# QuantEcon/dynamic_factor_models

Measured on NVIDIA H100. Metric: EM iters/sec (N=200,r=8,T=500), higher is better.
Workload: dtype f64

## Files before the change

dynamic_factor_models_b200/csrc/dfm_api.cu:

```cuda
#include "../../include/dfm_b200.h"
#include "dfm_common.cuh"
#include "dfm_kernels_np.cuh"
#include "dfm_kernels_em.cuh"
#include "dfm_kernels_emb.cuh"
#include "dfm_kernels_ss.cuh"
#include "dfm_kernels_fused.cuh"
#include "dfm_kernels_fused2.cuh"
#include "dfm_kernels_als_masked.cuh"
#include "dfm_kernels_rep.cuh"
#include "dfm_kernels_inst.cuh"
#include <algorithm>
#include <new>
#include <thread>
#include <type_traits>
#include <vector>
#ifndef DFM_EMU
#include <dlfcn.h>
#else
#include <map>
#include <mutex>
#endif

#ifdef DFM_EMU
typedef int cudaError_t;
// ... 24 lines not shown
static inline cudaError_t cudaFree(void* p) { free(p); return 0; }
static inline cudaError_t cudaMemcpyAsync(void* d, const void* s, size_t n, cudaMemcpyKind, cudaStream_t) { memcpy(d, s, n); return 0; }
static inline cudaError_t cudaMemsetAsync(void* d, int v, size_t n, cudaStream_t) { memset(d, v, n); return 0; }
static inline cudaError_t cudaMemcpy2DAsync(void* d, size_t dp, const void* s, size_t sp, size_t w, size_t rows, cudaMemcpyKind, cudaStream_t) {
  for (size_t j = 0; j < rows; ++j) memcpy((char*)d + j * dp, (const char*)s + j * sp, w);
  return 0;
}
static inline cudaError_t cudaStreamCreate(cudaStream_t* s) { *s = nullptr; return 0; }
static inline cudaError_t cudaStreamDestroy(cudaStream_t) { return 0; }
static inline cudaError_t cudaStreamSynchronize(cudaStream_t) { return 0; }
static inline cudaError_t cudaSetDevice(int) { return 0; }
static inline cudaError_t cudaGetDeviceCount(int* n) { *n = 1; return 0; }
static inline cudaError_t cudaGetLastError() { cudaError_t e = g_emu_last_err; g_emu_last_err = cudaSuccess; return e; }
static inline const char* cudaGetErrorString(cudaError_t e) {
  return e == cudaErrorInvalidConfiguration ? "emu: launch past a device limit (grid, block or shared memory)"
       : e == cudaErrorInvalidValue ? "emu: shared-memory attribute past the device limit" : "emu";
}
#define DFM_SET_SMEM(kern, bytes) emu_set_smem((const void*)(kern), (size_t)(bytes))
#else
#define DFM_SET_SMEM(kern, bytes) cudaFuncSetAttribute(kern, cudaFuncAttributeMaxDynamicSharedMemorySize, (int)(bytes))
#endif

using namespace dfm;

struct ProfRec { const char* name; 
#ifndef DFM_EMU
  cudaEvent_t e0, e1;
#endif
};

struct dfm_handle {
  int device;
  int nsm;
  cudaStream_t stream;
  cudaStream_t copy_stream;
  cudaStream_t d2h_stream;
  int* done_host; int* done_dev; size_t done_cap;
  int* pinned_one;
  bool own_stream;
  char* ws;
  size_t ws_bytes;
  long long launches;
  int profile;
  std::vector<ProfRec>* prof;
  char err[256];
};

namespace {

const size_t kMaxSmem = 220 * 1024;
const int kMaxReadyChunks = 4096;
const int kMaxGridBatch = 65535;

struct Arena {
  char* base; size_t off;
  explicit Arena(char* b) : base(b), off(0) {}
  template <typename Tp> Tp* get(size_t n) {
    size_t bytes = (n * sizeof(Tp) + 255) & ~(size_t)255;
    Tp* p = base ? reinterpret_cast<Tp*>(base + off) : nullptr;
    off += bytes;
    return p;
  }
};

int fail(dfm_handle* h, int code, const char* msg) {
  if (h) { snprintf(h->err, sizeof(h->err), "%s", msg); }
// ... 92 lines not shown
  cuuint64_t strides[1] = {(cuuint64_t)T * 8};
  cuuint32_t box[2] = {F2_TS, 8 * F2_SBS}, es[2] = {1, 1};
  CUresult rc = fn(out, CU_TENSOR_MAP_DATA_TYPE_FLOAT64, 2, (void*)X, dims, strides, box, es, CU_TENSOR_MAP_INTERLEAVE_NONE,
                   CU_TENSOR_MAP_SWIZZLE_NONE, CU_TENSOR_MAP_L2_PROMOTION_L2_256B, CU_TENSOR_MAP_FLOAT_OOB_FILL_NONE);
  if (rc != CUDA_SUCCESS) { snprintf(h->err, sizeof(h->err), "cuTensorMapEncodeTiled failed (%d)", (int)rc); return DFM_ERR_CUDA; }
  return DFM_OK;
#endif
}

template <int Lo, int Hi, typename F>
static auto dispatch(int v, F&& f) {
  if constexpr (Lo == Hi) return f(std::integral_constant<int, Lo>{});
  else {
    if (v == Lo) return f(std::integral_constant<int, Lo>{});
    return dispatch<Lo + 1, Hi>(v, f);
  }
}

template <typename K>
static int resident_grid(const dfm_handle* h, K kern, int threads, size_t smem, int B) {
#ifdef DFM_EMU
  (void)threads;
  DFM_SET_SMEM(kern, smem);
  return std::min(B, h->nsm * 8);
#else
  DFM_SET_SMEM(kern, smem);
  int occ = 1;
  cudaOccupancyMaxActiveBlocksPerMultiprocessor(&occ, kern, threads, smem);
  if (occ < 1) occ = 1;
  return std::min(B, h->nsm * occ);
#endif
}

static int launch_em_fused(dfm_handle* h, const FusedArgs& fa, int r, bool use2) {
  return dispatch<1, 8>(r, [&](auto R) -> int {
    constexpr int RT = decltype(R)::value;
    if (use2) {
      const size_t smem = fused2_smem_doubles<RT>(fa.T, fa.N) * 8;
      const int grid = resident_grid(h, k_em_fused2<RT>, 256, smem, fa.B);
      CUtensorMap tm; int rc = make_panel_tmap(h, fa.X, fa.T, (long long)fa.B * fa.N, &tm); if (rc) return rc;
      L(k_em_fused2<RT>, grid, 1, 256, smem, fa, tm);
    } else {
      const size_t smem = fused_smem_doubles<RT>(fa.T, fa.N) * 8;
      const int grid = resident_grid(h, k_em_fused<RT>, 128, smem, fa.B);
      L(k_em_fused<RT>, grid, 1, 128, smem, fa);
    }
    return DFM_OK;
  });
}

struct EmbPlan {
  bool on; int ncb, ntE, nsE, nper, ntM, tsM, tper;
  double *Bpart, *qpart, *Spart, *sxxpart, *Cpart; int* counters;
  size_t smE, smM;
};
static EmbPlan emb_plan(int T, int N, int r, int batch, int nsm) {
  EmbPlan e{};
  e.on = r <= 32;
  if (!e.on) return e;
  e.ncb = (r + 7) / 8;
  const int target = 2 * nsm;
  e.ntE = (T + EMB_TILE - 1) / EMB_TILE;
  int want = (target + e.ntE * batch - 1) / (e.ntE * batch);
  int ns = std::max((N + EMB_MAXSPLIT - 1) / EMB_MAXSPLIT, std::min(want, (N + 31) / 32));
  e.nper = (((N + ns - 1) / ns) + 3) & ~3;
  e.nsE = (N + e.nper - 1) / e.nper;
  e.ntM = (N + EMB_TILE - 1) / EMB_TILE;
  want = (target + e.ntM * batch - 1) / (e.ntM * batch);
  int ts = std::max(1, std::min(want, (T + 31) / 32));
  e.tper = (((T + ts - 1) / ts) + 3) & ~3;
  e.tsM = (T + e.tper - 1) / e.tper;
  if ((long long)e.nsE * batch > 65535 || (long long)e.tsM * batch > 65535) { e.on = false; return e; }
// ... 118 lines not shown
  int n_missing = batch;
  if (emb.on) {
    L(k_em_count_missing, 1, 1, 128, 48 * 8, d.st, batch, d.active);
    CK(cudaMemcpyAsync(&n_missing, d.active, sizeof(int), cudaMemcpyDeviceToHost, h->stream));
    CK(cudaStreamSynchronize(h->stream));
    CK(cudaMemsetAsync(emb.counters, 0, sizeof(int) * (size_t)batch * (emb.ntE + emb.ntM), h->stream));
  }
  const bool any_missing = n_missing > 0, any_bal = emb.on ? (n_missing < batch) : true;
  const int emb_on = emb.on ? 1 : 0;
  int h_active = batch;
  for (int it = 0; it < mi && h_active > 0; ++it) {
    if (any_missing) L(k_em_contract, nblkC, batch, ntC, ((size_t)(np + r) * ntC + 8) * 8, x, d.L, g.W, d.R, g.logR, g.C, T, N, r, g.Bt, g.qt, g.slr, g.nt, g.Ct, d.st);
    if (any_bal) {
      if (!emb.on) L(k_em_contract_bal, (T + 31) / 32, batch, 256, 8 * 32 * 3 * 8, x, g.W, d.R, g.logR, T, N, r, g.Bt, g.qt, g.slr, g.nt, d.st);
      else emb_launch_E(h, emb, x, g.W, d.R, g.logR, T, N, r, batch, g.Bt, g.qt, g.slr, g.nt, d.st);
    }
    launch_filter_smooth(h, ncl, g, batch, T, r, p, d.A, d.Q, d.P0, d.Fs, d.PsF, d.ll, d.st, mi, o->tol, want_psf);
    if (any_missing || !emb.on) L(k_em_mstep_series, N, batch, 64, (size_t)(2 * np + r + 8) * 8, x, d.Fs, d.PsF, g.Sff, T, N, r, d.L, d.R, d.st, emb_on);
    if (any_bal && emb.on) {
      emb_launch_M(h, emb, x, d.Fs, g.Sff, T, N, r, batch, d.L, d.R, g.W, g.logR, d.st);
      L(k_emb_close, batch, 1, 256, 0, N, r, p, emb.ntM, emb.Cpart, g.C, d.A, g.An, d.Q, g.Qn, d.st, mi, 1);
    }
    if (any_missing || !emb.on) L(k_em_prep, batch, 1, 128, 0, d.L, d.R, N, r, p, g.W, g.logR, g.C, d.A, g.An, d.Q, g.Qn, d.st, mi, 1, emb_on);
    if (o->tol > 0 && ((it & 3) == 3)) {
      L(k_em_count_active, 1, 1, 128, 48 * 8, d.st, batch, d.active);
      CK(cudaMemcpyAsync(&h_active, d.active, sizeof(int), cudaMemcpyDeviceToHost, h->stream));
      CK(cudaStreamSynchronize(h->stream));
    }
  }
  L(k_em_collect, batch, 1, 1, 0, d.st, d.it, d.stat);
  return DFM_OK;
}

static int launch_als_fused2(dfm_handle* h, const AlsFusedArgs& fa, int r) {
  return dispatch<1, 8>(r, [&](auto R) -> int {
    constexpr int RT = decltype(R)::value;
    const size_t smem = als_fused2_smem_doubles<RT>(fa.T, fa.N) * 8;
    const int grid = resident_grid(h, k_als_fused2<RT>, 256, smem, fa.B);
    CUtensorMap tm; int rc = make_panel_tmap(h, fa.Xs, fa.T, (long long)fa.B * fa.N, &tm); if (rc) return rc;
    L(k_als_fused2<RT>, grid, 1, 256, smem, fa, tm);
    return DFM_OK;
  });
}
static void launch_als_masked(dfm_handle* h, const AlsMaskedArgs& fa, int r) {
  dispatch<1, 8>(r, [&](auto R) {
    constexpr int RT = decltype(R)::value;
    const size_t smem = als_masked_smem_doubles<RT>(fa.T, fa.N) * 8;
    const int grid = resident_grid(h, k_als_masked<RT>, 256, smem, fa.B);
    L(k_als_masked<RT>, grid, 1, 256, smem, fa);
  });
}
static bool als_masked_shape_ok(int T, int N, int r) {
  if (r < 1 || r > 8) return false;
  return ((size_t)r * (T | 1) + (size_t)r * (N | 1) + 5 * (size_t)r * r + 48) * 8 <= 100 * 1024;
}
static bool als_fused2_shape_ok(int T, int N, int r) {
  if (r < 1 || r > 8 || T < 4 || (T & 1)) return false;
  return ((size_t)FZ * pad4mod16(T) + (size_t)r * pad4mod16(N) + (size_t)N + 4 * (size_t)r * r + 2 * r + 48 +
          2 * F2_NCW * 72 + (size_t)F2_S * F2_STG + 32) * 8 <= 113 * 1024;
}

static bool fused2_shape_ok(int T, int N, int r, int p) {
  if (p != 1 || r < 1 || r > 8 || T < 4 || (T & 1)) return false;
  size_t need = ((size_t)FZ * pad4mod16(T) + (size_t)r * pad4mod16(N) + 3 * (size_t)N + 30 * (size_t)r * r + 2 * (size_t)r +
                 std::max((size_t)97 * r + (size_t)r * r, (size_t)2 * F2_NCW * 72) + (size_t)F2_S * F2_STG + 106) * 8;
  return need <= 113 * 1024;
}

static bool fused_shape_ok(int T, int N, int r, int p) {
  if (p != 1 || r < 1 || r > 8 || T < 3) return false;
  return ((size_t)FZ * pad4mod16(T) + (size_t)r * pad4mod16(N) + 3 * (size_t)N + 31 * (size_t)r * r + 66 * (size_t)r + 128) * 8 <= kMaxSmem;
// ... 128 lines not shown
    case DFM_ERR_CUDA: return "CUDA error / no device";
    case DFM_ERR_UNSUPPORTED: return "unsupported problem size";
    case DFM_ERR_NCCL: return "NCCL error";
  }
  return "unknown";
}

static void handle_teardown(dfm_handle* h) {
  if (!h) return;
  if (h->stream) cudaStreamSynchronize(h->stream);
  if (h->ws) cudaFree(h->ws);
  if (h->own_stream && h->stream) cudaStreamDestroy(h->stream);
#ifndef DFM_EMU
  if (h->copy_stream) { cudaStreamSynchronize(h->copy_stream); cudaStreamDestroy(h->copy_stream); }
  if (h->pinned_one) cudaFreeHost(h->pinned_one);
  if (h->d2h_stream) { cudaStreamSynchronize(h->d2h_stream); cudaStreamDestroy(h->d2h_stream); }
  if (h->done_host) cudaFreeHost(h->done_host);
  if (h->prof) for (auto& r : *h->prof) { cudaEventDestroy(r.e0); cudaEventDestroy(r.e1); }
#endif
  delete h->prof;
  delete h;
}

int dfm_create_on_stream(int device, void* cuda_stream, dfm_handle** out) {
  if (!out) return DFM_ERR_ARG;
  *out = nullptr;
  int ndev = 0;
  if (cudaGetDeviceCount(&ndev) != cudaSuccess || ndev <= 0 || device < 0 || device >= ndev) return DFM_ERR_CUDA;
  if (cudaSetDevice(device) != cudaSuccess) return DFM_ERR_CUDA;
  dfm_handle* h = new (std::nothrow) dfm_handle();
  if (!h) return DFM_ERR_CUDA;
  h->device = device; h->ws = nullptr; h->ws_bytes = 0; h->launches = 0; h->err[0] = 0;
  h->nsm = 132;
  h->profile = 0; h->prof = new std::vector<ProfRec>();
  h->stream = nullptr; h->own_stream = false;
  h->copy_stream = nullptr; h->pinned_one = nullptr; h->d2h_stream = nullptr; h->done_host = nullptr; h->done_dev = nullptr; h->done_cap = 0;
#ifndef DFM_EMU
  if (cudaDeviceGetAttribute(&h->nsm, cudaDevAttrMultiProcessorCount, device) != cudaSuccess || h->nsm <= 0) { handle_teardown(h); return DFM_ERR_CUDA; }
  if (cudaStreamCreateWithFlags(&h->copy_stream, cudaStreamNonBlocking) != cudaSuccess) { h->copy_stream = nullptr; handle_teardown(h); return DFM_ERR_CUDA; }
  if (cudaStreamCreateWithFlags(&h->d2h_stream, cudaStreamNonBlocking) != cudaSuccess) { h->d2h_stream = nullptr; handle_teardown(h); return DFM_ERR_CUDA; }
  if (cudaHostAlloc((void**)&h->pinned_one, sizeof(int), cudaHostAllocDefault) != cudaSuccess) { h->pinned_one = nullptr; handle_teardown(h); return DFM_ERR_CUDA; }
  *h->pinned_one = 1;
#endif
  if (cuda_stream) { h->stream = (cudaStream_t)cuda_stream; h->own_stream = false; }
  else { if (cudaStreamCreate(&h->stream) != cudaSuccess) { h->stream = nullptr; handle_teardown(h); return DFM_ERR_CUDA; } h->own_stream = true; }
  DFM_SET_SMEM(k_em_filter_smooth, kMaxSmem); DFM_SET_SMEM(k_als_factor, kMaxSmem); DFM_SET_SMEM(k_em_contract, kMaxSmem);
  DFM_SET_SMEM(k_lyapunov, kMaxSmem); DFM_SET_SMEM(k_var, kMaxSmem); DFM_SET_SMEM(k_pca_finish, kMaxSmem);
  DFM_SET_SMEM(k_jacobi, kMaxSmem); DFM_SET_SMEM(k_subspace_eig, kMaxSmem); DFM_SET_SMEM(k_loading, kMaxSmem); DFM_SET_SMEM(k_als_lambda, kMaxSmem);
  if (cudaGetLastError() != cudaSuccess) { handle_teardown(h); return DFM_ERR_CUDA; }
  *out = h;
  return DFM_OK;
}
int dfm_create(int device, dfm_handle** out) { return dfm_create_on_stream(device, nullptr, out); }

int dfm_destroy(dfm_handle* h) {
  if (!h) return DFM_ERR_ARG;
  cudaSetDevice(h->device);
  handle_teardown(h);
  return DFM_OK;
}
int dfm_sync(dfm_handle* h) { if (!h) return DFM_ERR_ARG; CK(cudaStreamSynchronize(h->stream)); return DFM_OK; }
long long dfm_launch_count(const dfm_handle* h) { return h ? h->launches : -1; }
const char* dfm_last_error(const dfm_handle* h) { return h ? h->err : "null handle"; }

int dfm_profile_enable(dfm_handle* h, int on) {
  if (!h) return DFM_ERR_ARG;
  h->profile = on ? 1 : 0;
  return DFM_OK;
}
int dfm_profile_query(dfm_handle* h, const char* name, double* ms, long long* count) {
  if (!h || !ms || !count) return DFM_ERR_ARG;
// ... 753 lines not shown
```

dynamic_factor_models_b200/csrc/dfm_kernels_fused.cuh:

```cuda
#pragma once
#include "dfm_common.cuh"

namespace dfm {

#define FZ 8
#define ZI(t_, i_) ((i_) * Tp + (t_))
#define LI(n_, c_) ((c_) * Np + (n_))
__host__ __device__ inline int pad4mod16(int x) { return x + ((4 - x % 16) + 16) % 16; }

struct FusedArgs {
  const double* X;
  double* Lam;
  double* R;
  double* A;
  double* Q;
  const double* P0;
  double* Fs;
  double* PsF;
  double* loglik;
  int* iters; int* status;
  double* scratch;
  int B, T, N, max_iter;
  double tol;
  const int* ready; int ready_chunk;
  int* done;
  double* P0out;
  int p0_steps;
};
#define FUSED_SCR(R_) (5 * (R_) * (R_) + 1)

__device__ __forceinline__ double w_max(double v) {
#ifndef DFM_EMU
  for (int o = 16; o > 0; o >>= 1) v = fmax(v, __shfl_xor_sync(0xffffffffu, v, o));
#endif
  return v;
}

#ifdef DFM_EMU
#define DFM_HELPER inline
#else
#define DFM_HELPER __device__ __noinline__
#endif
template <int R>
DFM_HELPER void w_gemm(double* C, const double* A, bool ta, const double* B, bool tb) {
#ifndef DFM_EMU
  if (R == 8) {
    const int lane = threadIdx.x & 31, lr = lane >> 2, lc = lane & 3;
    double d0 = 0.0, d1 = 0.0;
#pragma unroll
    for (int kc = 0; kc < 2; ++kc) {
      const int kk = 4 * kc + lc;
      const double av = ta ? A[kk * 8 + lr] : A[lr * 8 + kk];
      const double bv = tb ? B[lr * 8 + kk] : B[kk * 8 + lr];
      asm volatile("mma.sync.aligned.m8n8k4.row.col.f64.f64.f64.f64 {%0,%1}, {%2}, {%3}, {%0,%1};\n"
                   : "+d"(d0), "+d"(d1) : "d"(av), "d"(bv));
    }
    C[lr * 8 + 2 * lc] = d0; C[lr * 8 + 2 * lc + 1] = d1;
    __syncwarp();
    return;
  }
// ... 659 lines not shown
```

dynamic_factor_models_b200/csrc/dfm_kernels_fused2.cuh:

```cuda
#pragma once
#include <algorithm>
#include "dfm_kernels_fused.cuh"
#ifdef DFM_EMU
struct CUtensorMap { char opaque[128]; };
#define DFM_GRID_CONSTANT
#else
#include <cuda.h>
#define DFM_GRID_CONSTANT __grid_constant__
#endif

namespace dfm {

#ifndef F2_SBS
#define F2_SBS 1
#endif
#ifndef F2_S
#define F2_S (4 / F2_SBS)
#endif
#define F2_STG (F2_SBS * 8 * F2_TS)
#ifndef F2_TC
#define F2_TC 132
#endif
#define F2_TS F2_TC
#define F2_NCW 6
#define F2_GPARTS_S 4
#define F2_GPARTS ((R == 8) ? (F2_NCW + 1) : F2_GPARTS_S)
#define F2_NRB (((F2_TC + 7) / 8 + F2_NCW - 1) / F2_NCW)
#define F2_NKC (((F2_TC + 3) / 4 + F2_NCW - 1) / F2_NCW)
static_assert(F2_TC % 16 == 4 || F2_TC % 16 == 12, "ring pitch must be 4 or 12 mod 16");
static_assert(F2_TC <= 256 && (F2_TC * 64) % 128 == 0, "TMA box / stage alignment");
#define F2_NEXS(R_) ((F2_S * F2_STG - 4 * (R_) * (R_)) / FUSED_SCR(R_))
#define F2_RTAIL(R_) (F2_S * F2_STG - 4 * (R_) * (R_))

#ifndef DFM_EMU
__device__ __forceinline__ uint32_t f2_smem_u32(const void* p) { return (uint32_t)__cvta_generic_to_shared(p); }
__device__ __forceinline__ void f2_mbar_init(uint64_t* bar, int cnt) { asm volatile("mbarrier.init.shared::cta.b64 [%0], %1;" ::"r"(f2_smem_u32(bar)), "r"(cnt)); }
__device__ __forceinline__ void f2_mbar_expect(uint64_t* bar, uint32_t bytes) { asm volatile("mbarrier.arrive.expect_tx.shared::cta.b64 _, [%0], %1;" ::"r"(f2_smem_u32(bar)), "r"(bytes) : "memory"); }
__device__ __forceinline__ void f2_mbar_arrive(uint64_t* bar) { asm volatile("mbarrier.arrive.shared::cta.b64 _, [%0];" ::"r"(f2_smem_u32(bar)) : "memory"); }
__device__ __forceinline__ void f2_mbar_wait(uint64_t* bar, uint32_t phase) {
  asm volatile("{\n.reg .pred p;\nWAIT_%=:\nmbarrier.try_wait.parity.shared::cta.b64 p, [%0], %1;\n@p bra DONE_%=;\nbra WAIT_%=;\nDONE_%=:\n}" ::"r"(f2_smem_u32(bar)), "r"(phase) : "memory");
}
__device__ __forceinline__ void f2_tma_2d(void* dst, const CUtensorMap* tmap, int x, int y, uint64_t* bar) {
  asm volatile("cp.async.bulk.tensor.2d.shared::cluster.global.mbarrier::complete_tx::bytes [%0], [%1, {%2, %3}], [%4];"
               ::"r"(f2_smem_u32(dst)), "l"(reinterpret_cast<uint64_t>(tmap)), "r"(x), "r"(y), "r"(f2_smem_u32(bar)) : "memory");
}
#endif


#ifndef DFM_EMU
struct F2Ring {
  double* ring; uint64_t* full; uint64_t* empty;
  int rs; uint32_t rph; bool wrap;
  __device__ __forceinline__ void advance() { if (++rs == F2_S) { rs = 0; rph ^= 1; wrap = true; } }
  __device__ __forceinline__ void skip(long long n) { for (long long q = 0; q < n; ++q) advance(); }
};

__device__ __forceinline__ void f2_produce(F2Ring& rg, const CUtensorMap* tmap, int row0, int T, int N, bool c_outer) {
  const int lane = threadIdx.x & 31;
  const int nsb = (N + 8 * F2_SBS - 1) / (8 * F2_SBS), nck = (T + F2_TC - 1) / F2_TC;
  const int n_out = c_outer ? nck : nsb, n_in = c_outer ? nsb : nck;
  for (int o = 0; o < n_out; ++o)
    for (int i = 0; i < n_in; ++i) {
      const int c = c_outer ? o : i, sb = c_outer ? i : o;
      if (rg.wrap) f2_mbar_wait(&rg.empty[rg.rs], rg.rph ^ 1);
      if (lane == 0) {
        f2_mbar_expect(&rg.full[rg.rs], (uint32_t)(F2_STG * 8));
        f2_tma_2d(rg.ring + (size_t)rg.rs * F2_STG, tmap, c * F2_TC, row0 + sb * 8 * F2_SBS, &rg.full[rg.rs]);
      }
      __syncwarp();
      rg.advance();
    }
}

template <int R>
__device__ __forceinline__ double f2_consume_E(F2Ring& rg, int cw, int T, int N, int Tp, int Np, double* Z, const double* Lam,
                                               const double* rinv) {
  const int lane = threadIdx.x & 31, lr = lane >> 2, lc = lane & 3;
  const int nsg = (N + 8 * F2_SBS - 1) / (8 * F2_SBS), nck = (T + F2_TC - 1) / F2_TC;
  double qacc = 0.0;
  for (int c = 0; c < nck; ++c) {
    const int len = (T - c * F2_TC < F2_TC) ? T - c * F2_TC : F2_TC;
    double d[F2_NRB][2][2];
#pragma unroll
    for (int j = 0; j < F2_NRB; ++j) { d[j][0][0] = 0.0; d[j][0][1] = 0.0; d[j][1][0] = 0.0; d[j][1][1] = 0.0; }
    for (int sg = 0; sg < nsg; ++sg) {
      f2_mbar_wait(&rg.full[rg.rs], rg.rph);
      const double* stage = rg.ring + (size_t)rg.rs * F2_STG;
#pragma unroll
      for (int sub = 0; sub < F2_SBS; ++sub) {
        const double* tile = stage + (size_t)sub * 8 * F2_TS;
        const int sb = sg * F2_SBS + sub;
        double rn[2], lm[2], av[2][F2_NRB];
#pragma unroll
        for (int kc = 0; kc < 2; ++kc) {
          const int n = sb * 8 + kc * 4 + lc;
          const bool nok = n < N;
          rn[kc] = nok ? (rinv ? rinv[n] : 1.0) : 0.0;
          lm[kc] = (nok && lr < R) ? Lam[LI(n, lr)] : 0.0;
          const double* trow = tile + (kc * 4 + lc) * F2_TS + lr;
#pragma unroll
// ... 139 lines not shown
  ring += ((128u - (f2_smem_u32(ring) & 127u)) & 127u) / 8;
#endif
  double* gscr = a.scratch + (size_t)DFM_BX * T * FUSED_SCR(R);
#define GSC(t_) (gscr + (size_t)(t_) * FUSED_SCR(R))
#define SCRP(t_) (((t_) < F2_NEXS(R)) ? (ring + (size_t)(t_) * FUSED_SCR(R)) : (gscr + (size_t)(t_) * FUSED_SCR(R)))
#define GPS(t_) (gscr + (size_t)(t_) * FUSED_SCR(R) + 4 * RR)
#ifndef DFM_EMU
  __shared__ uint64_t fullb[F2_S], emptyb[F2_S];
  if (threadIdx.x == 0) { for (int s_ = 0; s_ < F2_S; ++s_) { f2_mbar_init(&fullb[s_], 1); f2_mbar_init(&emptyb[s_], F2_NCW); } }
  asm volatile("fence.mbarrier_init.release.cluster;" ::: "memory");
  __syncthreads();
  F2Ring rg; rg.ring = ring; rg.full = fullb; rg.empty = emptyb; rg.rs = 0; rg.rph = 0; rg.wrap = false;
#endif
  const double eps = 1e-14;

  for (int b = DFM_BX; b < a.B; b += DFM_GX) {
    const double* X = a.X + (size_t)b * T * N;
#ifndef DFM_EMU
    if (a.ready) {
      if (threadIdx.x == 0) {
        const int* f_ = a.ready + b / a.ready_chunk; int v_ = 0;
        for (;;) { asm volatile("ld.acquire.sys.global.s32 %0, [%1];" : "=r"(v_) : "l"(f_) : "memory"); if (v_) break; __nanosleep(256); }
      }
      __syncthreads();
    }
#endif
    for (int e = DFM_TID; e < N * R; e += DFM_NT) { int i = e % N, c = e / N; Lam[LI(i, c)] = a.Lam[(size_t)b * N * R + e]; }
    for (int e = DFM_TID; e < N; e += DFM_NT) Rv[e] = a.R[(size_t)b * N + e];
    for (int e = DFM_TID; e < RR; e += DFM_NT) {
      int i = e / R, j = e % R;
      M[e] = a.A[(size_t)b * RR + i + R * j]; Q[e] = a.Q[(size_t)b * RR + i + R * j];
    }
    if (DFM_TID == 0) ctl[2] = 0;
    DFM_SYNC();
    if (a.P0out || a.ready) {
      for (int e = DFM_TID; e < a.max_iter; e += DFM_NT) a.loglik[(size_t)b * a.max_iter + e] = DFM_NAN;
      if (a.P0out) {
        for (int e = DFM_TID; e < RR; e += DFM_NT) { Pp[e] = Q[e]; Pi[e] = M[e]; }
        DFM_SYNC();
        for (int s_ = 0; s_ < a.p0_steps; ++s_) {
          for (int e = DFM_TID; e < RR; e += DFM_NT) { const int i = e / R, j = e % R; double v = 0.0; for (int l = 0; l < R; ++l) v += Pi[i * R + l] * Pp[l * R + j]; Wm[e] = v; }
          DFM_SYNC();
          for (int e = DFM_TID; e < RR; e += DFM_NT) { const int i = e / R, j = e % R; double v = 0.0; for (int l = 0; l < R; ++l) v += Wm[i * R + l] * Pi[j * R + l]; G[e] = v; }
          DFM_SYNC();
          for (int e = DFM_TID; e < RR; e += DFM_NT) {
            const int i = e / R, j = e % R; double v = 0.0; for (int l = 0; l < R; ++l) v += Pi[i * R + l] * Pi[l * R + j];
            Wm[e] = v; Pp[e] = Pp[e] + 1.0 * G[e];
          }
          DFM_SYNC();
          for (int e = DFM_TID; e < RR; e += DFM_NT) Pi[e] = Wm[e];
          DFM_SYNC();
        }
        for (int e = DFM_TID; e < RR; e += DFM_NT) { const int i = e / R, j = e % R; if (i > j) { const double v = 0.5 * (Pp[i * R + j] + Pp[j * R + i]); Pp[i * R + j] = v; Pp[j * R + i] = v; } }
        DFM_SYNC();
        for (int e = DFM_TID; e < RR; e += DFM_NT) { const int i = e / R, j = e % R; a.P0out[(size_t)b * RR + i + R * j] = Pp[e]; }
      }
      DFM_SYNC();
    }
    int it = 0, status = 0;
    double ll_prev = 0.0;
    for (; it < a.max_iter; ++it) {
      double slr_p = 0.0;
      for (int i = DFM_TID; i < N; i += DFM_NT) { double rv = Rv[i]; rinv[i] = 1.0 / rv; slr_p += log(rv); if (!(rv > 0.0)) ctl[2] = 1; }
      slr_p = block_sum(slr_p, red);
      if (DFM_TID == 0) scal[0] = slr_p;
      DFM_SYNC();
// ... 137 lines not shown
          bool conv = frozen && t > lo && dmax <= eps * pmax;
          for (int e = DFM_LANE; e < RR; e += DFM_WSZ) Psn[e] = Ps[e];
          DFM_WSYNC();
          if (conv) {
            tb = t;
            double cnt = (double)(t - lo);
            w_gemm<R>(T1, Ps, false, Jinf, true);
            for (int e = DFM_LANE; e < RR; e += DFM_WSZ) {
              SPall[e] += cnt * Ps[e]; SP00[e] += cnt * Ps[e];
              SPff2[e] += ((lo >= 1) ? cnt : cnt - 1.0) * Ps[e];
              SP11[e] += cnt * T1[e];
              Ppinf[e] = Ps[e];
            }
            DFM_WSYNC();
            t = lo - 1;
          } else --t;
        }
        if (DFM_LANE == 0) ctl[1] = tb;
        DFM_WSYNC();
      };
      double qacc = 0.0;
#ifdef DFM_EMU
      for (int t = 0; t < T; ++t) {
        for (int c = 0; c < FZ; ++c) Z[ZI(t, c)] = 0.0;
        for (int n = 0; n < N; ++n) {
          double x = X[(size_t)n * T + t], xr = x * rinv[n];
          qacc += x * xr;
          for (int c = 0; c < R; ++c) Z[ZI(t, c)] += xr * Lam[LI(n, c)];
        }
      }
#else
      {
        const long long nitems = (long long)((N + 8 * F2_SBS - 1) / (8 * F2_SBS)) * ((T + F2_TC - 1) / F2_TC);
        if (DFM_WARP == 0) f2_produce(rg, &tmap, b * N, T, N, true);
        else if (DFM_WARP <= F2_NCW) qacc += f2_consume_E<R>(rg, DFM_WARP - 1, T, N, Tp, Np, Z, Lam, rinv);
        else {
          rg.skip(nitems);
          chain_fwd();
        }
      }
#endif
#ifdef DFM_EMU
      chain_fwd();
      chain_bwd();
#endif
      DFM_SYNC();
      const int nE = ctl[0], frozen = ctl[3];
#ifndef DFM_EMU
      if (DFM_WARP == F2_NCW + 1) chain_bwd();
      else
#endif
      {
      {
        const int ncp = (nE < F2_NEXS(R)) ? nE : F2_NEXS(R);
        for (int e = F2_PTID; e < ncp * FUSED_SCR(R); e += F2_PNT) ring[e] = gscr[e];
        if (frozen) for (int e = F2_PTID; e < 4 * RR; e += F2_PNT) ring[F2_RTAIL(R) + e] = GSC(T - 1)[e];
      }
      for (int t = nE + F2_PTID; t < T; t += F2_PNT) {
        double bb[R], u[R];
#pragma unroll
        for (int j = 0; j < R; ++j) bb[j] = Z[ZI(t, j)];
#pragma unroll
        for (int i = 0; i < R; ++i) { double s = 0.0;
#pragma unroll
          for (int j = 0; j < R; ++j) s += Pfinf[i * R + j] * bb[j]; u[i] = s; }
#pragma unroll
        for (int i = 0; i < R; ++i) Z[ZI(t, i)] = u[i];
// ... 184 lines not shown

        for (int e = DFM_LANE; e < RR; e += DFM_WSZ) T1[e] = Sm[e] + SPall[e];
        DFM_WSYNC();
        w_sym<R>(T1);
        w_inv<R>(G, T1, tmp, bad);
        for (int e = DFM_LANE; e < RR; e += DFM_WSZ) {
          int i = e / R, j = e % R;
          Pp[e] = Sm[e] - Z[ZI(T - 1, i)] * Z[ZI(T - 1, j)] + SP00[e];
          Pi[e] = Sm[e] - Z[ZI(0, i)] * Z[ZI(0, j)] + SPff2[e];
          Pf[e] = S11m[e] + SP11[e];
        }
        DFM_WSYNC();
        w_sym<R>(Pp);
        w_inv<R>(Wm, Pp, tmp, bad);
        w_gemm<R>(Phi, Pf, false, Wm, false);
        w_gemm<R>(Pn, Phi, false, Pf, true);
        for (int e = DFM_LANE; e < RR; e += DFM_WSZ) Pn[e] = (Pi[e] - Pn[e]) / (double)(T - 1);
        DFM_WSYNC();
        w_sym<R>(Pn);
      };
#ifdef DFM_EMU
      for (int n = 0; n < N; ++n) {
        double s2 = 0.0, acc[R];
        for (int c = 0; c < R; ++c) acc[c] = 0.0;
        for (int t = 0; t < T; ++t) { double x = X[(size_t)n * T + t]; s2 += x * x; for (int c = 0; c < R; ++c) acc[c] += x * Z[ZI(t, c)]; }
        for (int c = 0; c < R; ++c) Lam[LI(n, c)] = acc[c];
        sxx[n] = s2;
      }
#else
      {
        asm volatile("fence.proxy.async.shared::cta;" ::: "memory");
        __syncthreads();
        const long long nitems = (long long)((N + 8 * F2_SBS - 1) / (8 * F2_SBS)) * ((T + F2_TC - 1) / F2_TC);
        if (DFM_WARP == 0) f2_produce(rg, &tmap, b * N, T, N, false);
        else if (DFM_WARP <= F2_NCW) f2_consume_M<R>(rg, DFM_WARP - 1, T, N, Tp, Np, Z, Lam, sxx, part);
        else {
          rg.skip(nitems);
          mstep_small();
        }
      }
#endif
#ifdef DFM_EMU
      mstep_small();
#endif
      DFM_SYNC();
      DFM_SYNC();
      for (int n = DFM_TID; n < N; n += DFM_NT) {
        double sx[R], lam[R];
#pragma unroll
        for (int c = 0; c < R; ++c) sx[c] = Lam[LI(n, c)];
        double q1 = 0.0, q2 = 0.0;
#pragma unroll
        for (int i = 0; i < R; ++i) { double s = 0.0;
#pragma unroll
          for (int j = 0; j < R; ++j) s += G[i * R + j] * sx[j]; lam[i] = s; q1 += s * sx[i]; }
#pragma unroll
        for (int i = 0; i < R; ++i) { double s = 0.0;
#pragma unroll
          for (int j = 0; j < R; ++j) s += T1[i * R + j] * lam[j]; q2 += lam[i] * s; }
#pragma unroll
        for (int c = 0; c < R; ++c) Lam[LI(n, c)] = lam[c];
        Rv[n] = (sxx[n] - 2.0 * q1 + q2) / (double)T;
      }
      DFM_SYNC();
      for (int e = DFM_TID; e < RR; e += DFM_NT) { M[e] = Phi[e]; Q[e] = Pn[e]; }
      if (DFM_TID == 0) a.loglik[(size_t)b * a.max_iter + it] = ll;
      DFM_SYNC();
      if (ctl[2] || !(ll == ll)) { status = 3; ++it; break; }
      bool conv = (it >= 1) && fabs(ll - ll_prev) <= a.tol * 0.5 * (fabs(ll) + fabs(ll_prev));
      ll_prev = ll;
      if (conv) { ++it; break; }
    }
    for (int e = DFM_TID; e < N * R; e += DFM_NT) { int i = e % N, c = e / N; a.Lam[(size_t)b * N * R + e] = Lam[LI(i, c)]; }
    for (int e = DFM_TID; e < N; e += DFM_NT) a.R[(size_t)b * N + e] = Rv[e];
    for (int e = DFM_TID; e < RR; e += DFM_NT) {
      int i = e % R, j = e / R;
      a.A[(size_t)b * RR + e] = M[i * R + j]; a.Q[(size_t)b * RR + e] = Q[i * R + j];
    }
    for (int e = DFM_TID; e < T * R; e += DFM_NT) { int t = e % T, c = e / T; a.Fs[(size_t)b * T * R + e] = Z[ZI(t, c)]; }
    {
      const int nE = ctl[0], tb = ctl[1], frozen = ctl[3];
      const int lo = frozen ? nE - 1 : T;
      for (int e = DFM_TID; e < T * NP; e += DFM_NT) {
        int t = e % T, pe = e / T;
        int i = 0; while ((i + 1) * (i + 2) / 2 <= pe) ++i;
        int j = pe - i * (i + 1) / 2;
        bool in_frozen = frozen && tb >= 0 && t >= lo && t < tb;
        double v = in_frozen ? Ppinf[i * R + j] : GPS(t)[i * R + j];
        a.PsF[(size_t)b * T * NP + e] = v;
      }
    }
    if (DFM_TID == 0) { a.iters[b] = it > a.max_iter ? a.max_iter : it; a.status[b] = status; }
#ifndef DFM_EMU
    if (a.done) __threadfence_system();
#endif
    DFM_SYNC();
#ifndef DFM_EMU
    if (a.done && threadIdx.x == 0) *(volatile int*)(a.done + b) = 1;
#endif
  }
}

#undef SCRP
#undef GSC
#undef GPS
struct AlsFusedArgs {
  const double* Xs;
  double* F;
  double* Lam;
  AlsState* st;
  int B, T, N;
  double tol;
  long long max_iter;
};

template <int R>
__global__ void DFM_FUSED2_BOUNDS k_als_fused2(AlsFusedArgs a, const DFM_GRID_CONSTANT CUtensorMap tmap) {
  DFM_SMEM(sm);
  constexpr int RR = R * R;
  const int T = a.T, N = a.N;
  const int Tp = pad4mod16(T), Np = pad4mod16(N);
  double* Z = sm;
  double* Lam = Z + (size_t)FZ * Tp;
  double* sxx = Lam + (size_t)R * Np;
  double* FtF = sxx + N;  double* Gi = FtF + RR;  double* LtL = Gi + RR;  double* Hi = LtL + RR;
  double* tmp = Hi + RR;
  double* red = tmp + 2 * R;
  int* ctl = (int*)(red + 40);
  double* part = red + 48;
  double* ring = part + 2 * F2_NCW * 72;
#ifndef DFM_EMU
  ring += ((128u - (f2_smem_u32(ring) & 127u)) & 127u) / 8;
  __shared__ uint64_t fullb[F2_S], emptyb[F2_S];
  if (threadIdx.x == 0) { for (int s_ = 0; s_ < F2_S; ++s_) { f2_mbar_init(&fullb[s_], 1); f2_mbar_init(&emptyb[s_], F2_NCW); } }
  asm volatile("fence.mbarrier_init.release.cluster;" ::: "memory");
  __syncthreads();
  F2Ring rg; rg.ring = ring; rg.full = fullb; rg.empty = emptyb; rg.rs = 0; rg.rph = 0; rg.wrap = false;
  const long long nitems = (long long)((N + 8 * F2_SBS - 1) / (8 * F2_SBS)) * ((T + F2_TC - 1) / F2_TC);
#endif
  for (int b = DFM_BX; b < a.B; b += DFM_GX) {
    const double* X = a.Xs + (size_t)b * T * N;
    for (int e = DFM_TID; e < FZ * Tp; e += DFM_NT) Z[e] = 0.0;
    DFM_SYNC();
    for (int e = DFM_TID; e < T * R; e += DFM_NT) { int t = e % T, c = e / T; Z[ZI(t, c)] = a.F[(size_t)b * T * R + e]; }
    if (DFM_TID == 0) ctl[0] = 0;
    DFM_SYNC();
    double ssr = 0.0, ssr_old = 0.0;
    long long it = 0;
    int status = 0;
    while (it < a.max_iter) {
      for (int e = DFM_TID; e < RR; e += DFM_NT) {
        int i = e / R, j = e % R; double s = 0.0;
        for (int t = 0; t < T; ++t) s += Z[ZI(t, i)] * Z[ZI(t, j)];
        FtF[e] = s;
      }
      DFM_SYNC();
      if (DFM_WARP == 0) w_inv<R>(Gi, FtF, tmp, &ctl[0]);
#ifdef DFM_EMU
      for (int n = 0; n < N; ++n) {
        double s2 = 0.0, acc[R];
        for (int c = 0; c < R; ++c) acc[c] = 0.0;
        for (int t = 0; t < T; ++t) { double x = X[(size_t)n * T + t]; s2 += x * x; for (int c = 0; c < R; ++c) acc[c] += x * Z[ZI(t, c)]; }
        for (int c = 0; c < R; ++c) Lam[LI(n, c)] = acc[c];
        sxx[n] = s2;
      }
#else
      if (DFM_WARP == 0) f2_produce(rg, &tmap, b * N, T, N, false);
      else if (DFM_WARP <= F2_NCW) f2_consume_M<R>(rg, DFM_WARP - 1, T, N, Tp, Np, Z, Lam, sxx, part);
      else rg.skip(nitems);
#endif
      DFM_SYNC();
      for (int n = DFM_TID; n < N; n += DFM_NT) {
        double sx[R], lam[R];
#pragma unroll
        for (int c = 0; c < R; ++c) sx[c] = Lam[LI(n, c)];
#pragma unroll
        for (int i = 0; i < R; ++i) { double s = 0.0;
#pragma unroll
          for (int j = 0; j < R; ++j) s += Gi[i * R + j] * sx[j]; lam[i] = s; }
#pragma unroll
        for (int c = 0; c < R; ++c) Lam[LI(n, c)] = lam[c];
      }
      DFM_SYNC();
      for (int e = DFM_TID; e < RR; e += DFM_NT) {
        int i = e / R, j = e % R; double s = 0.0;
        for (int n = 0; n < N; ++n) s += Lam[LI(n, i)] * Lam[LI(n, j)];
        LtL[e] = s;
      }
      DFM_SYNC();
      if (DFM_WARP == 0) w_inv<R>(Hi, LtL, tmp, &ctl[0]);
      double tssp = 0.0;
#ifdef DFM_EMU
      for (int t = 0; t < T; ++t) {
        for (int c = 0; c < FZ; ++c) Z[ZI(t, c)] = 0.0;
        for (int n = 0; n < N; ++n) { double x = X[(size_t)n * T + t]; tssp += x * x; for (int c = 0; c < R; ++c) Z[ZI(t, c)] += x * Lam[LI(n, c)]; }
      }
#else
      if (DFM_WARP == 0) f2_produce(rg, &tmap, b * N, T, N, true);
      else if (DFM_WARP <= F2_NCW) tssp += f2_consume_E<R>(rg, DFM_WARP - 1, T, N, Tp, Np, Z, Lam, nullptr);
      else rg.skip(nitems);
#endif
      DFM_SYNC();
      double bf = 0.0;
      for (int t = DFM_TID; t < T; t += DFM_NT) {
        double bb[R], f[R];
#pragma unroll
        for (int j = 0; j < R; ++j) bb[j] = Z[ZI(t, j)];
#pragma unroll
        for (int i = 0; i < R; ++i) { double s = 0.0;
#pragma unroll
          for (int j = 0; j < R; ++j) s += Hi[i * R + j] * bb[j]; f[i] = s; bf += s * bb[i]; }
#pragma unroll
        for (int i = 0; i < R; ++i) Z[ZI(t, i)] = f[i];
      }
      bf = block_sum(bf, red);
      tssp = block_sum(tssp, red);
      ssr_old = ssr; ssr = tssp - bf;
      ++it;
      if (ctl[0]) { status = 3; break; }
      if (!(fabs(ssr_old - ssr) >= a.tol * (double)T * (double)N)) break;
      if (it >= a.max_iter) { status = 4; break; }
    }
    for (int e = DFM_TID; e < T * R; e += DFM_NT) { int t = e % T, c = e / T; a.F[(size_t)b * T * R + e] = Z[ZI(t, c)]; }
    for (int e = DFM_TID; e < N * R; e += DFM_NT) { int i = e % N, c = e / N; a.Lam[(size_t)b * N * R + e] = Lam[LI(i, c)]; }
    if (DFM_TID == 0) { a.st[b].ssr_old = ssr_old; a.st[b].ssr = ssr; a.st[b].iters = (int)it; a.st[b].done = 1; a.st[b].status = status; }
    DFM_SYNC();
  }
}

template <int R>
inline size_t als_fused2_smem_doubles(int T, int N) {
  return (size_t)FZ * pad4mod16(T) + (size_t)R * pad4mod16(N) + (size_t)N + 4 * (size_t)R * R + 2 * R + 48 +
         2 * F2_NCW * 72 + (size_t)F2_S * F2_STG + 26;
}

template <int R>
inline size_t fused2_smem_doubles(int T, int N) {
  return (size_t)FZ * pad4mod16(T) + (size_t)R * pad4mod16(N) + 3 * (size_t)N + 30 * (size_t)R * R + 2 * R + 40 + 8 + 8 +
         std::max((size_t)97 * R + (size_t)R * R, (size_t)2 * F2_NCW * 72) + (size_t)F2_S * F2_STG + 26;
}

}
```

Before: 1.581 million.

## Pin leading panel stripes in L2 with TMA cache hints across EM iterations

```diff
diff --git a/dynamic_factor_models_b200/csrc/dfm_api.cu b/dynamic_factor_models_b200/csrc/dfm_api.cu
--- a/dynamic_factor_models_b200/csrc/dfm_api.cu
+++ b/dynamic_factor_models_b200/csrc/dfm_api.cu
@@ -80,6 +80,7 @@
 struct dfm_handle {
   int device;
   int nsm;
+  int l2_bytes;
   cudaStream_t stream;
   cudaStream_t copy_stream;
   cudaStream_t d2h_stream;
@@ -238,12 +239,21 @@
 #endif
 }
 
-static int launch_em_fused(dfm_handle* h, const FusedArgs& fa, int r, bool use2) {
+static void l2_keep_plan(const dfm_handle* h, int grid, int B, int T, int N, int keep[2]) {
+  const long long budget = (long long)h->l2_bytes * F2_L2KEEP_PCT / 100, group = 64LL * F2_SBS * T;
+  const long long nsg = (N + 8 * F2_SBS - 1) / (8 * F2_SBS);
+  const int tail = (B % grid) ? B % grid : grid;
+  keep[0] = (int)std::min(nsg, budget / (grid * group));
+  keep[1] = (int)std::min(nsg, budget / (tail * group));
+}
+
+static int launch_em_fused(dfm_handle* h, FusedArgs fa, int r, bool use2) {
   return dispatch<1, 8>(r, [&](auto R) -> int {
     constexpr int RT = decltype(R)::value;
     if (use2) {
       const size_t smem = fused2_smem_doubles<RT>(fa.T, fa.N) * 8;
       const int grid = resident_grid(h, k_em_fused2<RT>, 256, smem, fa.B);
+      l2_keep_plan(h, grid, fa.B, fa.T, fa.N, fa.l2_keep);
       CUtensorMap tm; int rc = make_panel_tmap(h, fa.X, fa.T, (long long)fa.B * fa.N, &tm); if (rc) return rc;
       L(k_em_fused2<RT>, grid, 1, 256, smem, fa, tm);
     } else {
@@ -428,11 +438,12 @@
   return DFM_OK;
 }
 
-static int launch_als_fused2(dfm_handle* h, const AlsFusedArgs& fa, int r) {
+static int launch_als_fused2(dfm_handle* h, AlsFusedArgs fa, int r) {
   return dispatch<1, 8>(r, [&](auto R) -> int {
     constexpr int RT = decltype(R)::value;
     const size_t smem = als_fused2_smem_doubles<RT>(fa.T, fa.N) * 8;
     const int grid = resident_grid(h, k_als_fused2<RT>, 256, smem, fa.B);
+    l2_keep_plan(h, grid, fa.B, fa.T, fa.N, fa.l2_keep);
     CUtensorMap tm; int rc = make_panel_tmap(h, fa.Xs, fa.T, (long long)fa.B * fa.N, &tm); if (rc) return rc;
     L(k_als_fused2<RT>, grid, 1, 256, smem, fa, tm);
     return DFM_OK;
@@ -627,11 +638,13 @@
   if (!h) return DFM_ERR_CUDA;
   h->device = device; h->ws = nullptr; h->ws_bytes = 0; h->launches = 0; h->err[0] = 0;
   h->nsm = 132;
+  h->l2_bytes = 50 << 20;
   h->profile = 0; h->prof = new std::vector<ProfRec>();
   h->stream = nullptr; h->own_stream = false;
   h->copy_stream = nullptr; h->pinned_one = nullptr; h->d2h_stream = nullptr; h->done_host = nullptr; h->done_dev = nullptr; h->done_cap = 0;
 #ifndef DFM_EMU
   if (cudaDeviceGetAttribute(&h->nsm, cudaDevAttrMultiProcessorCount, device) != cudaSuccess || h->nsm <= 0) { handle_teardown(h); return DFM_ERR_CUDA; }
+  if (cudaDeviceGetAttribute(&h->l2_bytes, cudaDevAttrL2CacheSize, device) != cudaSuccess) { handle_teardown(h); return DFM_ERR_CUDA; }
   if (cudaStreamCreateWithFlags(&h->copy_stream, cudaStreamNonBlocking) != cudaSuccess) { h->copy_stream = nullptr; handle_teardown(h); return DFM_ERR_CUDA; }
   if (cudaStreamCreateWithFlags(&h->d2h_stream, cudaStreamNonBlocking) != cudaSuccess) { h->d2h_stream = nullptr; handle_teardown(h); return DFM_ERR_CUDA; }
   if (cudaHostAlloc((void**)&h->pinned_one, sizeof(int), cudaHostAllocDefault) != cudaSuccess) { h->pinned_one = nullptr; handle_teardown(h); return DFM_ERR_CUDA; }
diff --git a/dynamic_factor_models_b200/csrc/dfm_kernels_fused.cuh b/dynamic_factor_models_b200/csrc/dfm_kernels_fused.cuh
--- a/dynamic_factor_models_b200/csrc/dfm_kernels_fused.cuh
+++ b/dynamic_factor_models_b200/csrc/dfm_kernels_fused.cuh
@@ -26,6 +26,7 @@
   int* done;
   double* P0out;
   int p0_steps;
+  int l2_keep[2];
 };
 #define FUSED_SCR(R_) (5 * (R_) * (R_) + 1)
 
diff --git a/dynamic_factor_models_b200/csrc/dfm_kernels_fused2.cuh b/dynamic_factor_models_b200/csrc/dfm_kernels_fused2.cuh
--- a/dynamic_factor_models_b200/csrc/dfm_kernels_fused2.cuh
+++ b/dynamic_factor_models_b200/csrc/dfm_kernels_fused2.cuh
@@ -31,6 +31,9 @@
 static_assert(F2_TC <= 256 && (F2_TC * 64) % 128 == 0, "TMA box / stage alignment");
 #define F2_NEXS(R_) ((F2_S * F2_STG - 4 * (R_) * (R_)) / FUSED_SCR(R_))
 #define F2_RTAIL(R_) (F2_S * F2_STG - 4 * (R_) * (R_))
+#ifndef F2_L2KEEP_PCT
+#define F2_L2KEEP_PCT 55
+#endif
 
 #ifndef DFM_EMU
 __device__ __forceinline__ uint32_t f2_smem_u32(const void* p) { return (uint32_t)__cvta_generic_to_shared(p); }
@@ -40,9 +43,20 @@
 __device__ __forceinline__ void f2_mbar_wait(uint64_t* bar, uint32_t phase) {
   asm volatile("{\n.reg .pred p;\nWAIT_%=:\nmbarrier.try_wait.parity.shared::cta.b64 p, [%0], %1;\n@p bra DONE_%=;\nbra WAIT_%=;\nDONE_%=:\n}" ::"r"(f2_smem_u32(bar)), "r"(phase) : "memory");
 }
-__device__ __forceinline__ void f2_tma_2d(void* dst, const CUtensorMap* tmap, int x, int y, uint64_t* bar) {
-  asm volatile("cp.async.bulk.tensor.2d.shared::cluster.global.mbarrier::complete_tx::bytes [%0], [%1, {%2, %3}], [%4];"
-               ::"r"(f2_smem_u32(dst)), "l"(reinterpret_cast<uint64_t>(tmap)), "r"(x), "r"(y), "r"(f2_smem_u32(bar)) : "memory");
+__device__ __forceinline__ void f2_tma_2d(void* dst, const CUtensorMap* tmap, int x, int y, uint64_t* bar, uint64_t policy) {
+  asm volatile("cp.async.bulk.tensor.2d.shared::cluster.global.mbarrier::complete_tx::bytes.L2::cache_hint [%0], [%1, {%2, %3}], [%4], %5;"
+               ::"r"(f2_smem_u32(dst)), "l"(reinterpret_cast<uint64_t>(tmap)), "r"(x), "r"(y), "r"(f2_smem_u32(bar)), "l"(policy) : "memory");
+}
+
+__device__ __forceinline__ int f2_keep_stages(const int* keep, int B, int b) {
+  const int G = (int)gridDim.x;
+  return (b / G < B / G) ? keep[0] : keep[1];
+}
+__device__ __forceinline__ void f2_release(const double* X, long long row0, int keep, int T, long long rows) {
+  const long long r1 = min(row0 + 8LL * F2_SBS * keep, rows);
+  const uintptr_t a0 = reinterpret_cast<uintptr_t>(X + row0 * T) & ~(uintptr_t)127, a1 = reinterpret_cast<uintptr_t>(X + r1 * T);
+  for (uintptr_t p = a0 + (uintptr_t)threadIdx.x * 128; p < a1; p += (uintptr_t)blockDim.x * 128)
+    asm volatile("applypriority.L2::evict_normal [%0], 128;" ::"l"(p) : "memory");
 }
 #endif
 
@@ -55,17 +69,20 @@
   __device__ __forceinline__ void skip(long long n) { for (long long q = 0; q < n; ++q) advance(); }
 };
 
-__device__ __forceinline__ void f2_produce(F2Ring& rg, const CUtensorMap* tmap, int row0, int T, int N, bool c_outer) {
+__device__ __forceinline__ void f2_produce(F2Ring& rg, const CUtensorMap* tmap, int row0, int T, int N, bool c_outer, const int* keep) {
   const int lane = threadIdx.x & 31;
   const int nsb = (N + 8 * F2_SBS - 1) / (8 * F2_SBS), nck = (T + F2_TC - 1) / F2_TC;
-  const int n_out = c_outer ? nck : nsb, n_in = c_outer ? nsb : nck;
+  const int n_out = c_outer ? nck : nsb, n_in = c_outer ? nsb : nck, nkeep = *keep;
+  uint64_t pol_last, pol_first;
+  asm volatile("createpolicy.fractional.L2::evict_last.b64 %0, 1.0;" : "=l"(pol_last));
+  asm volatile("createpolicy.fractional.L2::evict_first.b64 %0, 1.0;" : "=l"(pol_first));
   for (int o = 0; o < n_out; ++o)
     for (int i = 0; i < n_in; ++i) {
       const int c = c_outer ? o : i, sb = c_outer ? i : o;
       if (rg.wrap) f2_mbar_wait(&rg.empty[rg.rs], rg.rph ^ 1);
       if (lane == 0) {
         f2_mbar_expect(&rg.full[rg.rs], (uint32_t)(F2_STG * 8));
-        f2_tma_2d(rg.ring + (size_t)rg.rs * F2_STG, tmap, c * F2_TC, row0 + sb * 8 * F2_SBS, &rg.full[rg.rs]);
+        f2_tma_2d(rg.ring + (size_t)rg.rs * F2_STG, tmap, c * F2_TC, row0 + sb * 8 * F2_SBS, &rg.full[rg.rs], sb < nkeep ? pol_last : pol_first);
       }
       __syncwarp();
       rg.advance();
@@ -271,6 +288,9 @@
       M[e] = a.A[(size_t)b * RR + i + R * j]; Q[e] = a.Q[(size_t)b * RR + i + R * j];
     }
     if (DFM_TID == 0) ctl[2] = 0;
+#ifndef DFM_EMU
+    if (DFM_TID == 0) ctl[4] = f2_keep_stages(a.l2_keep, a.B, b);
+#endif
     DFM_SYNC();
     if (a.P0out || a.ready) {
       for (int e = DFM_TID; e < a.max_iter; e += DFM_NT) a.loglik[(size_t)b * a.max_iter + e] = DFM_NAN;
@@ -474,7 +494,7 @@
 #else
       {
         const long long nitems = (long long)((N + 8 * F2_SBS - 1) / (8 * F2_SBS)) * ((T + F2_TC - 1) / F2_TC);
-        if (DFM_WARP == 0) f2_produce(rg, &tmap, b * N, T, N, true);
+        if (DFM_WARP == 0) f2_produce(rg, &tmap, b * N, T, N, true, &ctl[4]);
         else if (DFM_WARP <= F2_NCW) qacc += f2_consume_E<R>(rg, DFM_WARP - 1, T, N, Tp, Np, Z, Lam, rinv);
         else {
           rg.skip(nitems);
@@ -725,7 +745,7 @@
         asm volatile("fence.proxy.async.shared::cta;" ::: "memory");
         __syncthreads();
         const long long nitems = (long long)((N + 8 * F2_SBS - 1) / (8 * F2_SBS)) * ((T + F2_TC - 1) / F2_TC);
-        if (DFM_WARP == 0) f2_produce(rg, &tmap, b * N, T, N, false);
+        if (DFM_WARP == 0) f2_produce(rg, &tmap, b * N, T, N, false, &ctl[4]);
         else if (DFM_WARP <= F2_NCW) f2_consume_M<R>(rg, DFM_WARP - 1, T, N, Tp, Np, Z, Lam, sxx, part);
         else {
           rg.skip(nitems);
@@ -764,6 +784,9 @@
       ll_prev = ll;
       if (conv) { ++it; break; }
     }
+#ifndef DFM_EMU
+    f2_release(a.X, (long long)b * N, ctl[4], T, (long long)a.B * N);
+#endif
     for (int e = DFM_TID; e < N * R; e += DFM_NT) { int i = e % N, c = e / N; a.Lam[(size_t)b * N * R + e] = Lam[LI(i, c)]; }
     for (int e = DFM_TID; e < N; e += DFM_NT) a.R[(size_t)b * N + e] = Rv[e];
     for (int e = DFM_TID; e < RR; e += DFM_NT) {
@@ -805,6 +828,7 @@
   int B, T, N;
   double tol;
   long long max_iter;
+  int l2_keep[2];
 };
 
 template <int R>
@@ -837,6 +861,9 @@
     DFM_SYNC();
     for (int e = DFM_TID; e < T * R; e += DFM_NT) { int t = e % T, c = e / T; Z[ZI(t, c)] = a.F[(size_t)b * T * R + e]; }
     if (DFM_TID == 0) ctl[0] = 0;
+#ifndef DFM_EMU
+    if (DFM_TID == 0) ctl[1] = f2_keep_stages(a.l2_keep, a.B, b);
+#endif
     DFM_SYNC();
     double ssr = 0.0, ssr_old = 0.0;
     long long it = 0;
@@ -858,7 +885,7 @@
         sxx[n] = s2;
       }
 #else
-      if (DFM_WARP == 0) f2_produce(rg, &tmap, b * N, T, N, false);
+      if (DFM_WARP == 0) f2_produce(rg, &tmap, b * N, T, N, false, &ctl[1]);
       else if (DFM_WARP <= F2_NCW) f2_consume_M<R>(rg, DFM_WARP - 1, T, N, Tp, Np, Z, Lam, sxx, part);
       else rg.skip(nitems);
 #endif
@@ -889,7 +916,7 @@
         for (int n = 0; n < N; ++n) { double x = X[(size_t)n * T + t]; tssp += x * x; for (int c = 0; c < R; ++c) Z[ZI(t, c)] += x * Lam[LI(n, c)]; }
       }
 #else
-      if (DFM_WARP == 0) f2_produce(rg, &tmap, b * N, T, N, true);
+      if (DFM_WARP == 0) f2_produce(rg, &tmap, b * N, T, N, true, &ctl[1]);
       else if (DFM_WARP <= F2_NCW) tssp += f2_consume_E<R>(rg, DFM_WARP - 1, T, N, Tp, Np, Z, Lam, nullptr);
       else rg.skip(nitems);
 #endif
@@ -914,6 +941,9 @@
       if (!(fabs(ssr_old - ssr) >= a.tol * (double)T * (double)N)) break;
       if (it >= a.max_iter) { status = 4; break; }
     }
+#ifndef DFM_EMU
+    f2_release(a.Xs, (long long)b * N, ctl[1], T, (long long)a.B * N);
+#endif
     for (int e = DFM_TID; e < T * R; e += DFM_NT) { int t = e % T, c = e / T; a.F[(size_t)b * T * R + e] = Z[ZI(t, c)]; }
     for (int e = DFM_TID; e < N * R; e += DFM_NT) { int i = e % N, c = e / N; a.Lam[(size_t)b * N * R + e] = Lam[LI(i, c)]; }
     if (DFM_TID == 0) { a.st[b].ssr_old = ssr_old; a.st[b].ssr = ssr; a.st[b].iters = (int)it; a.st[b].done = 1; a.st[b].status = status; }
```

Result: faster. 1.658 million, median of 6 (+4.9%).
